# Newiz430/CellSegmentation

Measured on AMD Instinct MI355X. Metric: tiles/sec fwd+bwd (ResNet-50 MIL, 299x299), higher is better.
Workload: dtype bf16; 1 GPU; ResNet-50 tile classifier (train_tile.py --scratch semantics: fwd + CE + full bwd + Adam), bag=64 tiles of 299x299x3 per GPU, freeze_bn=True; tiles_per_gpu=64, parallelism=dp1

## Files before the change

### cellsegmentation_amd/_lib.py

```python
import ctypes
import os
from ctypes import POINTER, Structure, c_char_p, c_double, c_float, c_int, c_int32, c_int64, c_longlong, c_size_t, c_void_p

_HERE = os.path.dirname(os.path.abspath(__file__))
FLAVOUR = os.environ.get("CELLSEG_LIB_FLAVOUR", "")
if FLAVOUR not in ("", "ab"):
    raise RuntimeError(f"CELLSEG_LIB_FLAVOUR={FLAVOUR!r}: expected unset or 'ab'")
LIB_PATH = os.path.join(_HERE, f"libcellseg_hip_{FLAVOUR}.so" if FLAVOUR else "libcellseg_hip.so")

CS_F32, CS_BF16 = 0, 1
CS_ACT_NONE, CS_ACT_RELU, CS_ACT_SILU, CS_ACT_SIGMOID = 0, 1, 2, 3
CS_BN_BWD_OWN_RELU, CS_BN_BWD_FROZEN = 0x100, 0x200


class CsConvGeom(Structure):
    _fields_ = [(n, c_int32) for n in ("N", "H", "W", "C", "K", "R", "S", "stride", "pad", "P", "Q", "groups")]


class CsStageDesc(Structure):
    _fields_ = ([(n, c_void_p) for n in ("w", "gamma", "beta", "mean", "var", "conv_bias", "w_khwc", "w_chwk", "scale", "shift", "rstd")]
                + [("eps", c_float)] + [(n, c_int32) for n in ("K", "Cin", "R", "S", "Cp", "Kp", "block0", "fwd_packed", "bwd_packed")])


class CellsegLibraryMissing(RuntimeError):
# ... 15 lines not shown
    "cs_stage_conv_bn_multi": (c_int, [_P, c_int, c_int, c_int, _P]),
    "cs_stage_conv_bn_one": (c_int, [POINTER(CsStageDesc), c_int, _P]),
    "cs_weight_prep": (c_int, [_P, _P, c_int, c_int, c_int, c_int, c_int, c_int, c_int, _P, _P, _P]),
    "cs_conv2d_fwd": (c_int, [POINTER(CsConvGeom), c_int, _P, _P, _P, _P, _P, c_int, _P, _P, _P, _P]),
    "cs_conv2d_stats_workspace": (c_size_t, [c_longlong, c_int]),
    "cs_igemm_tile": (c_int, [c_longlong, c_int]),
    "cs_conv2d_dgrad": (c_int, [POINTER(CsConvGeom), c_int, _P, _P, _P, _P, _P, _P, _P, _P]),
    "cs_conv2d_fwd_bits": (c_int, [POINTER(CsConvGeom), c_int, _P, _P, _P, _P, _P, c_int, _P, _P, _P]),
    "cs_conv2d_dgrad_bits": (c_int, [POINTER(CsConvGeom), c_int, _P, _P, _P, _P, _P, _P, _P, _P]),
    "cs_conv2d_packed_supported": (c_int, [POINTER(CsConvGeom), c_int]),
    "cs_conv2d_packed_weight_bytes": (c_size_t, [POINTER(CsConvGeom), c_int]),
    "cs_pack_conv_weights": (c_int, [POINTER(CsConvGeom), c_int, _P, _P, _P]),
    "cs_conv2d_packed_partial_rows": (c_int, [POINTER(CsConvGeom), c_int]),
    "cs_conv2d_fwd_packed": (c_int, [POINTER(CsConvGeom), _P, _P, _P, _P, c_int, _P, _P, _P]),
    "cs_conv2d_dgrad_packed": (c_int, [POINTER(CsConvGeom), _P, _P, _P, c_int, _P, _P, _P, _P]),
    "cs_conv2d_wgrad": (c_int, [POINTER(CsConvGeom), c_int, _P, _P, _P, c_int, _P]),
    "cs_wgrad_finalize": (c_int, [_P, c_int, c_int, _P, _P, _P, _P, _P, c_int, c_int, c_int, c_int, c_int, _P, _P, _P, _P, _P, c_int, _P]),
    "cs_conv2d_wgrad_splits": (c_int, [POINTER(CsConvGeom), c_int]),
    "cs_weight_prep_grouped": (c_int, [_P, _P, c_int, c_int, c_int, c_int, c_int, _P, _P, _P]),
    "cs_conv2d_wgrad_batched_splits": (c_int, [POINTER(CsConvGeom), c_int, c_int]),
    "cs_conv2d_wgrad2_supported": (c_int, [POINTER(CsConvGeom), c_int]),
    "cs_conv2d_wgrad_batched": (c_int, [POINTER(CsConvGeom), c_int, _P, _P, _P, c_int, c_int, _P]),
    "cs_wgrad_finalize_batched": (c_int, [_P, _P, c_int, c_int, c_int, c_int, c_int, c_int, c_int, c_int, c_int, c_int, _P]),
    "cs_conv2d_dgrad_partial_rows": (c_int, [POINTER(CsConvGeom)]),
    "cs_fold_partial_rows": (c_int, [_P, c_int, c_int, _P, _P]),
    "cs_wgrad_finalize_grouped": (c_int, [_P, c_int, _P, _P, _P, _P, _P, c_int, c_int, c_int, c_int, _P, _P, _P, _P, _P]),
    "cs_colsum": (c_int, [_P, c_int, c_longlong, c_int, _P, _P]),
    "cs_colsum_partial_rows": (c_int, [c_longlong]),
    "cs_colsum_partial": (c_int, [_P, c_int, c_longlong, c_int, _P, _P]),
    "cs_positive_bits": (c_int, [_P, c_int, c_longlong, c_int, _P, _P]),
# ... 183 lines not shown
```

### cellsegmentation_amd/csrc/conv_v2.hip

```cpp
#include "cs_common.h"
#include <stdio.h>
#include <stdlib.h>
#include <utility>

namespace {

typedef int i32x4 __attribute__((ext_vector_type(4)));
typedef unsigned u32x4 __attribute__((ext_vector_type(4)));
constexpr unsigned OOB = 0x80000000u;

struct C2Params {
    const void* src;
    const void* wpk;
    void* dst;
    const float* shift;
    const void* residual;
    unsigned char* bits_out;
    const unsigned char* bits_in;
    float* slab;
    int act;
    int SH, SW, SC, NS;
    int DH, DW, NOUT;
    int Wp, Hp, PW, PH;
    int LW;
    int TH, TWl, tiles_x, tiles_y;
    unsigned n_tiles;
    int stride;
    int gather, GH, GWp;
    unsigned tap_sh[9];
    int lin;
    unsigned chunk_bytes;
    int add_stride, AH, AW;
    unsigned mg_dw, sh_dw, mg_dh, sh_dh, mg_wp, sh_wp, mg_hp, sh_hp;
    int NCC;
    int n_ntiles;
    unsigned M;
    unsigned src_bytes;
    unsigned pix_bytes;
    unsigned wpk_bytes;
};

__device__ __forceinline__ unsigned udivm(unsigned n, unsigned mg, unsigned sh) { return __umulhi(n, mg) >> sh; }

__device__ __forceinline__ i32x4 make_rsrc(const void* base, unsigned bytes) {
    const unsigned long long a = (unsigned long long)base;
    i32x4 r;
    r.x = (int)(unsigned)a;
    r.y = (int)((unsigned)(a >> 32) & 0xffffu);
    r.z = (int)bytes;
    r.w = 0x00020000;
    return r;
}
__device__ __forceinline__ unsigned lds_off(const void* p) { return (unsigned)(size_t)(__attribute__((address_space(3))) const unsigned char*)p; }

// ... 765 lines not shown
        wait_vm<0>();
        raw_barrier();
        epi.scr = smem_base + (unsigned)wave * EPI_WAVE;
    }
    asm volatile("s_nop 15\n\ts_nop 15\n\ts_nop 7");
    for_n<TM>([&]<int i>() {
        const f32x16 d = acc_read_w<i>();
        epi.template operator()<i>(d);
    });
    epi.finish();
    wait_vm<0>();
}

constexpr int R_MB = 96;

template <int TM, bool DG> struct RingEpilogue {
    static constexpr int E_OPS = 5 * TM + (DG ? 2 : 0);
    const C2Params& p;
    unsigned m0w = 0, m0w_next = 0xffffffffu, slab_row = 0;
    int n_w;
    bool alive;
    unsigned region;
    float sh[16];
    float s1[8];
    i32x4 q_res, q_bin;
    __amdgpu_buffer_rsrc_t r_dst, r_bout, r_slab;

    __device__ __forceinline__ RingEpilogue(const C2Params& p_, int n_w_, bool alive_, unsigned region_) : p(p_), n_w(n_w_), alive(alive_), region(region_) {}

    __device__ __forceinline__ unsigned piece() const {
        const unsigned lane = threadIdx.x & 63;
        return (lane & 3u) ^ ((lane >> 4) & 3u);
    }
    TileOffs cur, nxt;
    __device__ __forceinline__ void set_tile(unsigned base, unsigned base_next) {
        m0w = base; m0w_next = base_next;
        cur.set(base, alive, (unsigned)p.NOUT, (unsigned)n_w, piece(), p.M);
        nxt.set(base_next, alive, (unsigned)p.NOUT, (unsigned)n_w, piece(), p.M);
// ... 29 lines not shown

    __device__ __forceinline__ void prefetch(unsigned first_base) {
        const unsigned out_bytes = p.M * (unsigned)p.NOUT * 2u;
        r_dst = __builtin_amdgcn_make_buffer_rsrc(p.dst, 0, out_bytes, 0x00020000);
        r_bout = __builtin_amdgcn_make_buffer_rsrc(p.bits_out, 0, p.bits_out ? out_bytes >> 4 : 0u, 0x00020000);
        r_slab = __builtin_amdgcn_make_buffer_rsrc(p.slab, 0, p.slab ? 0x7ffffff0u : 0u, 0x00020000);
        q_res = make_rsrc(p.residual, !p.residual ? 0u : p.add_stride == 1 ? out_bytes : (unsigned)(p.NS * p.AH * p.AW * p.NOUT) * 2u);
        q_bin = make_rsrc(p.bits_in, p.bits_in ? out_bytes >> 4 : 0u);
        const int hh = (threadIdx.x & 63) >> 5;
#pragma unroll
        for (int g = 0; g < 4; ++g) {
            float4 s = make_float4(0.f, 0.f, 0.f, 0.f);
            if (!DG && p.shift && alive) s = *reinterpret_cast<const float4*>(p.shift + n_w + 8 * g + 4 * hh);
            sh[4 * g] = s.x; sh[4 * g + 1] = s.y; sh[4 * g + 2] = s.z; sh[4 * g + 3] = s.w;
        }
#pragma unroll
        for (int r = 0; r < 16; ++r) asm volatile("" : "+v"(sh[r]));
        TileOffs first;
        first.set(first_base, alive, (unsigned)p.NOUT, (unsigned)n_w, piece(), p.M);
        arm_all(first, std::make_integer_sequence<int, TM>{});
    }

    template <int I> __device__ __forceinline__ void operator()(const f32x16& acc) {
        const int lane = threadIdx.x & 63;
        const unsigned pc = piece();
        float v[16];
#pragma unroll
        for (int r = 0; r < 16; ++r) v[r] = DG ? acc[r] : acc[r] + sh[r];
        if (p.residual) {
            const uint4 xa = lds_get(acc_lds(I, 0)), xb = lds_get(acc_lds(I, 1));
            __builtin_amdgcn_wave_barrier();
            add_residual(v, xa, xb);
        }
        unsigned pk[8];
        pack_tile(v, !DG && p.act == CS_ACT_RELU, pk);
        lds_put(acc_lds(I, 0), make_uint4(pk[0], pk[1], pk[2], pk[3]));
        lds_put(acc_lds(I, 1), make_uint4(pk[4], pk[5], pk[6], pk[7]));
        __builtin_amdgcn_wave_barrier();
        uint4 o0 = lds_get(row_lds(I, 0)), o1 = lds_get(row_lds(I, 1));
        __builtin_amdgcn_wave_barrier();
        asm volatile("" : "+v"(o0.x), "+v"(o1.w));
        if constexpr (DG) {
            if (p.bits_in) {
                unsigned mbw;
// ... 24 lines not shown
                float a = s1[k];
                a += __shfl_xor(a, 4, 64);
                a += __shfl_xor(a, 8, 64);
                float t = a;
#pragma unroll
                for (int g = 1; g < 4; ++g) t += __shfl(a, ((lane & 3) ^ g) | (g << 4), 64);
                s1[k] = t;
            }
            const unsigned off = (lane < 4 && alive && p.slab) ? ((slab_row * 2u * (unsigned)p.NOUT + (unsigned)n_w + 8u * (unsigned)lane) * 4u) : OOB;
            __builtin_amdgcn_raw_buffer_store_b128(__builtin_bit_cast(u32x4, make_float4(s1[0], s1[1], s1[2], s1[3])), r_slab, off, 0, 0);
            __builtin_amdgcn_raw_buffer_store_b128(__builtin_bit_cast(u32x4, make_float4(s1[4], s1[5], s1[6], s1[7])), r_slab, off, 16, 0);
        }
    }
};

template <int TM, int WM, int WN, bool DG, bool GA = false>
__global__ __launch_bounds__(256, 2) __attribute__((amdgpu_num_vgpr(48))) void conv2_ring_kernel(C2Params p, int n_groups) {
    static_assert(WM * WN == 4 && WM * TM <= 4 && TM >= 2, "a ring slot holds up to 128 pixel rows");
    constexpr int BM = WM * TM * 32, BN = WN * 32;
    constexpr unsigned SLOT = 16384u, NSLOT = 3u, SLOT_ROWS = 128u;
    using Epi = RingEpilogue<TM, DG>;
    constexpr int E = Epi::E_OPS;
    static_assert(12 + 2 * E <= 63, "vmcnt field");
    extern __shared__ __attribute__((aligned(16))) unsigned char smem[];

    const int tid = threadIdx.x, lane = tid & 63;
    const int wave = __builtin_amdgcn_readfirstlane(tid >> 6);
    const int wm = wave / WN, wn = wave % WN;
    const int l31 = lane & 31, hh = lane >> 5;
    const WgTile wg(p);
    const unsigned group = wg.mtile;
    const int n_w = wg.n_w(p, BN, wn);
    const bool alive = n_w < p.NOUT;
    if (group * BM >= p.M) return;
    const int NCC = p.NCC;

    unsigned qb[4];
#pragma unroll
    for (int i = 0; i < 4; ++i) qb[i] = (unsigned)((wm * TM + (i < TM ? i : 0)) * 32 + l31);
    const i32x4 rsrc_a = make_rsrc(p.src, p.src_bytes);
    const i32x4 rsrc_b = make_rsrc(p.wpk, p.wpk_bytes);
    const unsigned smem_base = lds_off(smem);
    const unsigned hhb = (unsigned)hh * 256u;
    const unsigned cf0 = 0xf0u;
    const unsigned w_base = (unsigned)(n_w >> 5) * (unsigned)NCC * 4096u;

    int f_gy[2] = {0, 0}, f_gx[2] = {0, 0};
    auto tile_voff = [&](unsigned mt, unsigned (&vo)[2]) {
#pragma unroll
        for (int j = 0; j < 2; ++j) {
            const unsigned m = mt * BM + 16u * (unsigned)(wave + 4 * j) + (unsigned)(lane & 15);
            if (BM < 128 && 16 * (wave + 4 * j) >= BM) { vo[j] = OOB; continue; }
            if constexpr (GA) {
                const unsigned yall = udivm(m, p.mg_dw, p.sh_dw);
                const unsigned x = m - yall * (unsigned)p.DW;
                const unsigned n = udivm(yall, p.mg_dh, p.sh_dh);
                const unsigned y = yall - n * (unsigned)p.DH;
                vo[j] = (m < p.M && mt != 0xffffffffu) ? n * (unsigned)(p.GH * p.GWp) * 16u : 0xffffffffu;
                f_gy[j] = 2 * (int)y - 3;
                f_gx[j] = (int)x - 2;
                continue;
            }
            unsigned pix = m;
            if (p.stride > 1) {
                const unsigned yall = udivm(m, p.mg_dw, p.sh_dw);
                const unsigned x = m - yall * (unsigned)p.DW;
                const unsigned n = udivm(yall, p.mg_dh, p.sh_dh);
                const unsigned y = yall - n * (unsigned)p.DH;
                pix = (n * (unsigned)p.SH + y * (unsigned)p.stride) * (unsigned)p.SW + x * (unsigned)p.stride;
            }
            vo[j] = (m < p.M && mt != 0xffffffffu) ? pix * p.pix_bytes + (unsigned)(lane >> 4) * 16u : OOB;
        }
    };

    Epi epi(p, n_w, alive, smem_base + NSLOT * SLOT + (unsigned)wave * (unsigned)(TM * 2048));
    unsigned mt = group;
    epi.prefetch(mt * BM + (unsigned)(wm * TM * 32));
    asm volatile("; v[96:255] are owned by the main loop" ::: "v96", "v255");
    vzero_seq(std::make_integer_sequence<int, 16 * TM>{});

    unsigned f_mt = mt, f_slot = 0;
    int f_c = 0;
    unsigned f_vo[2];
    tile_voff(f_mt, f_vo);
    auto advance_fetch = [&]() {
        f_slot = f_slot == NSLOT - 1 ? 0u : f_slot + 1u;
        if (++f_c == NCC) {
            f_c = 0;
            if (f_mt != 0xffffffffu) {
                f_mt += (unsigned)n_groups;
                if (f_mt * BM >= p.M) f_mt = 0xffffffffu;
            }
            tile_voff(f_mt, f_vo);
        }
    };
    auto issue_b = [&]<int J>() {
        const unsigned bv = (alive && f_mt != 0xffffffffu) ? (unsigned)lane * 16u : OOB;
        bload4<J>(rsrc_b, bv, w_base + (unsigned)f_c * 4096u);
    };
    auto issue_a = [&]() {
        const unsigned dst = smem_base + f_slot * SLOT;
        if constexpr (GA) {
#pragma unroll
            for (int j = 0; j < 2; ++j) {
                auto slot_off = [&](int sl) -> unsigned {
                    const int kh = sl >> 2, pw = sl & 3;
                    const int iy = f_gy[j] + kh, px = f_gx[j] + pw;
                    const bool ok = f_vo[j] != 0xffffffffu && sl < 28 && (unsigned)iy < (unsigned)p.GH && (unsigned)px < (unsigned)p.GWp;
                    return ok ? f_vo[j] + (unsigned)(iy * p.GWp + px) * 16u : OOB;
                };
                const int s0 = f_c * 8 + (lane >> 4);
                dma_block2(rsrc_a, dst + (unsigned)(wave + 4 * j) * 2048u, slot_off(s0), slot_off(s0 + 4));
            }
            return;
        }
        dma_block(rsrc_a, dst + (unsigned)wave * 2048u, f_vo[0], (unsigned)f_c * 128u);
        dma_block(rsrc_a, dst + (unsigned)(wave + 4) * 2048u, f_vo[1], (unsigned)f_c * 128u);
    };
    issue_b.template operator()<0>(); issue_a(); advance_fetch();
    issue_b.template operator()<1>(); issue_a(); advance_fetch();
    int c = 0;
    unsigned slot = 0;
    bool fin1 = false, fin2 = false;
    auto step = [&]<int CUR>() -> bool {
        issue_b.template operator()<(CUR + 2) % 3>();
        const int nfin = (int)fin1 + (int)fin2;
        if (nfin == 0) wait_vm<12>();
        else if (nfin == 1) wait_vm<12 + E>();
        else wait_vm<12 + 2 * E>();
        raw_barrier();
        issue_a();
        advance_fetch();
        const unsigned sh_cur = slot * SLOT_ROWS;
        const bool fin = c == NCC - 1;
        bool more = true;
        if (!fin) {
            tap_mfma<TM, CUR, 0, 0u, 0u, true, false, true, false>(qb[0], qb[1], qb[2], qb[3], sh_cur, 0u, hhb, cf0);
            ++c;
        } else {
            const unsigned mt_next = mt + (unsigned)n_groups;
            const bool has_next = mt_next * BM < p.M;
            epi.set_tile(mt * BM + (unsigned)(wm * TM * 32), has_next ? mt_next * BM + (unsigned)(wm * TM * 32) : 0xffffffffu);
            epi.slab_row = mt * WM + wm;
            auto on_tile = [&]<int i>(const f32x16& d) {
                if (NCC == 1) wait_vm_mem<(E - 5 + 8 < 63 ? E - 5 + 8 : 63)>();
                else if (NCC == 2) wait_vm_mem<(E - 5 + 16 < 63 ? E - 5 + 16 : 63)>();
                epi.template operator()<i>(d);
            };
            tap_mfma<TM, CUR, 0, 0u, 0u, true, false, true, true>(qb[0], qb[1], qb[2], qb[3], sh_cur, 0u, hhb, cf0, on_tile);
            epi.finish();
            vzero_seq(std::make_integer_sequence<int, 16 * TM>{});
// ... 213 lines not shown
    static const int ring_tm = cs_env_int_("CELLSEG_RING_TM", 0);
    pl.tm = pl.kind == C2Kind::Ring22 ? 2 : (ring_tm >= 2 && ring_tm <= 4) ? ring_tm : pick_tm(p.M, p.n_ntiles);
    pl.nbw = 0;
    if (pl.kind == C2Kind::Ring14 && p.stride == 1 && !compact && p.NCC % 4 == 0) {
        const int wtm = pick_wide1_tm(p.M, p.n_ntiles, p.NCC);
        if (wtm) {
            pl.kind = C2Kind::Wide1x1; pl.tm = wtm; pl.nbw = wtm;
            p.lin = 1; p.chunk_bytes = 256u;
            p.tap_sh[0] = 0u; p.tap_sh[1] = 32u * (unsigned)wtm;
        }
    }
    pl.rows = partial_rows(pl);
    return true;
}

template <typename F, typename... Args>
int launch_kernel(F fn, const char* name, unsigned grid, size_t lds, hipStream_t st, const Args&... args) {
    if (!cs_allow_dynamic_lds_(reinterpret_cast<const void*>(fn), lds, lds > 81920 ? 163840 : 81920)) return CS_ERR_LAUNCH;
    cs_set_variant_(name);
    hipLaunchKernelGGL(fn, dim3(grid), dim3(256), lds, st, args...);
    CS_LAUNCH_CHECK();
    return CS_OK;
}
const char* tf(bool b) { return b ? "true" : "false"; }
unsigned xcd_grid(unsigned n_mt, int n_ntiles) { return ((n_mt + 7) / 8) * 8 * (unsigned)n_ntiles; }

template <int TM, int WM, int WN, bool DG>
int launch_ring_t(const C2Params& p, hipStream_t st) {
    const unsigned n_mt = (unsigned)cs_ceil_div(p.M, 32 * TM * WM);
    const unsigned best = ring_groups(n_mt, (unsigned)p.n_ntiles, nullptr);
    const size_t lds = 3 * 16384 + 4 * (size_t)TM * 2048;
    char name[64];
    snprintf(name, sizeof(name), "conv2_ring_kernel<%d,%d,%d,%s,%s>", TM, WM, WN, tf(DG), tf(p.gather));
    if constexpr (TM == 2 && !DG) {
        if (p.gather) return launch_kernel(conv2_ring_kernel<TM, WM, WN, DG, true>, name, best * (unsigned)p.n_ntiles, lds, st, p, (int)best);
    }
    if (p.gather) {
        cs_set_error_("conv2: gathered operand rows are served for 64 output channels only");
        return CS_ERR_UNSUPPORTED;
    }
    return launch_kernel(conv2_ring_kernel<TM, WM, WN, DG>, name, best * (unsigned)p.n_ntiles, lds, st, p, (int)best);
}

template <int TM, int WM, int WN, int NBW, bool DG, bool T2D = false>
int launch_halo_t(const C2Params& p, hipStream_t st) {
    const unsigned n_mt = T2D ? p.n_tiles : (unsigned)cs_ceil_div(p.M, 32 * TM * WM);
    const size_t lds = NBW != 8 && p.NCC > 1 ? (size_t)NBW * 8192 * 2 : (size_t)NBW * 8192 + EPI_LDS;
    char name[64];
    snprintf(name, sizeof(name), "conv2_halo_kernel<9,3,%d,%d,%d,%d,%s,%s>", TM, WM, WN, NBW, tf(DG), tf(T2D));
    return launch_kernel(conv2_halo_kernel<9, 3, TM, WM, WN, NBW, DG, T2D>, name, xcd_grid(n_mt, p.n_ntiles), lds, st, p);
}

template <int TM, int NBW, bool DG, int NTAP>
int launch_wide_t(const C2Params& p, hipStream_t st) {
    const unsigned n_mt = (unsigned)cs_ceil_div(p.M, 32 * TM);
    const size_t lds = (size_t)NBW * 8192 * (NTAP == 9 ? 2 : 3);
// ... 74 lines not shown
extern "C" int cs_conv2d_fwd_packed(const CsConvGeom* g, const void* x, const void* w_packed, const float* shift, const void* residual, int act,
                                    void* y, uint8_t* positive_bits, void* stream) {
    CS_CHECK_ARG(g && x && w_packed && y, "conv2d_fwd_packed: NULL tensor");
    CS_CHECK_ARG(act == CS_ACT_NONE || act == CS_ACT_RELU, "conv2d_fwd_packed: activation must be none or ReLU");
    C2Plan pl;
    if (!plan_any(g, 0, pl)) {
        cs_set_error_("conv2d_fwd_packed: geometry not served by the packed-operand kernel (ask cs_conv2d_packed_supported first)");
        return CS_ERR_UNSUPPORTED;
    }
    pl.p.src = x; pl.p.wpk = w_packed; pl.p.dst = y;
    pl.p.shift = shift; pl.p.residual = residual; pl.p.act = act;
    pl.p.bits_out = positive_bits;
    return launch_plan(pl, reinterpret_cast<hipStream_t>(stream), false);
}

extern "C" int cs_conv2d_dgrad_packed(const CsConvGeom* g, const void* dy, const void* w_packed, const void* add, int add_stride,
                                      const uint8_t* mask_bits, void* dx, float* partial_rows, void* stream) {
    CS_CHECK_ARG(g && dy && w_packed && dx, "conv2d_dgrad_packed: NULL tensor");
    CS_CHECK_ARG(add_stride == 1 || (add_stride == 2 && add), "conv2d_dgrad_packed: add_stride is 1, or 2 with a compact add operand");
    C2Plan pl;
    if (!plan_any(g, 1, pl)) {
        cs_set_error_("conv2d_dgrad_packed: geometry not served by the packed-operand kernel (ask cs_conv2d_packed_supported first)");
        return CS_ERR_UNSUPPORTED;
    }
    if (g->stride != 1)
        CS_CHECK_ARG(!add && !mask_bits && !partial_rows,
                     "conv2d_dgrad_packed: a strided 1x1 data gradient is written in compact [N][P][Q][C] form, without add / mask / column sums");
    if (add_stride == 2) {
        CS_CHECK_ARG(is_1x1(pl.kind) && pl.p.DH >= 2 && pl.p.DW >= 2, "conv2d_dgrad_packed: a strided add operand is served by the 1x1 kernels only");
        pl.p.add_stride = 2;
// ... 27 lines not shown
```

### cellsegmentation_amd/engine.py

```python
from collections import namedtuple
from types import SimpleNamespace

import torch

from . import _capture
from . import kernels as K

ACT_NONE, ACT_RELU, ACT_SILU = K.CS_ACT_NONE, K.CS_ACT_RELU, K.CS_ACT_SILU

PACKED = True
PACKED_TRAIN_BN = True
FUSE_STEM_POOL = True


class ConvUnit:
    kind = "conv"

    def __init__(self, name, conv, bn, act, src, dst, res=None):
        self.name, self.conv, self.bn, self.act = name, conv, bn, act
        self.src, self.dst, self.res = src, dst, res
        self.grouped = conv.groups != 1
        if self.grouped:
            cg = conv.in_channels // conv.groups
            if conv.in_channels != conv.out_channels or conv.in_channels % 64 != 0 or 64 % cg != 0 or conv.bias is not None:
                raise NotImplementedError(f"{name}: grouped convolution needs C == K, C % 64 == 0, (C/groups) | 64, no bias "
                                          "(the ResNeXt 32x4d / 32x8d 3x3 layers)")
        self._cache = None
# ... 4 lines not shown
            out.append(("bias", self.conv.bias))
        if self.bn is not None:
            out += [("gamma", self.bn.weight), ("beta", self.bn.bias)]
        return out

    def inputs(self):
        return [self.src] + ([self.res] if self.res is not None else [])

    def fwd(self, f, ui):
        x = f.t[self.src]
        N, H, W, Cp = x.shape
        conv = self.conv
        Kp = K.pad_channels(conv.out_channels)
        R, S = conv.kernel_size
        geom = K.make_geom(N, H, W, Cp, Kp, R, S, conv.stride[0], conv.padding[0])
        res = f.t[self.res] if self.res is not None else None
        batch_stats = _bn_uses_batch_stats(self.bn, f.bn_train)
        st = f.staged(ui, self, geom, batch_stats)
        stem = _is_paired_stem(self) and K.is_stem_geom(geom)
        xp = wp = None
        if ui == 0 and f.nchw_for_stem is not None:
            if not stem:
                raise RuntimeError("engine: the stem was expected to take the NCHW image (placeholder input would be read)")
            xp = K.stem_pair_from_nchw(f.nchw_for_stem, f.dtype)
        elif stem:
            xp = K.stem_pair_input(x)
        if stem:
            wp = K.stem_pair_weights(st.w_khwc)
        if batch_stats:
            stats = f.take_stats(Kp)
            if stem:
                z = K.stem_fwd(geom, xp, wp, None, st.shift, ACT_NONE, stats=stats)
            elif st.fwd_packed:
                z = K.conv_fwd_packed(geom, x, st.w_khwc, st.shift, None, ACT_NONE)
                K.bn_stats(z, stats)
            else:
                z = K.conv_fwd(geom, x, st.w_khwc, None, st.shift, None, ACT_NONE, stats=stats, grouped=self.grouped)
            y, mean, rstd = f.bn_train_fwd(self.bn, z, stats, res, self.act)
            f.aux[ui] = SimpleNamespace(geom=geom, st=st, train=True, z=z if f.save else None, mean=mean, rstd=rstd, xp=xp)
        else:
            want_bits = f.save and self.act == ACT_RELU
            pool_ui = None
            if stem and PACKED and FUSE_STEM_POOL and self.act == ACT_RELU and K.stem_pool_fwd_supported(geom, f.dtype):
                pool_ui = _sole_pool_consumer(f.plan, self)
            if pool_ui is not None:
                f.t[f.plan.units[pool_ui].dst], am = K.stem_pool_fwd(geom, xp, wp, st.shift, want_argmax=f.save)
                f.aux[pool_ui] = SimpleNamespace(argmax=am, in_hw=(geom.P, geom.Q))
                f.aux[ui] = SimpleNamespace(geom=geom, st=st, train=False, xp=xp)
                return
            if stem and PACKED and K.stem_fwd_packed_supported(geom, f.dtype):
                y = K.stem_fwd_packed(geom, xp, K.stem_pack_weights(wp), st.shift, self.act)
            elif stem:
                y = K.stem_fwd(geom, xp, wp, None, st.shift, self.act)
            elif st.fwd_packed and want_bits:
                y, f.bits[self.dst] = K.conv_fwd_packed(geom, x, st.w_khwc, st.shift, res, self.act, want_bits=True)
            elif st.fwd_packed:
# ... 248 lines not shown
def _is_paired_stem(u):
    if u.kind != "conv":
        return False
    c = u.conv
    return (not u.grouped and u.res is None and c.in_channels <= 3 and c.kernel_size == (7, 7)
            and c.stride == (2, 2) and c.padding == (3, 3))


def _sole_pool_consumer(plan, u):
    if plan.consumers.get(u.dst, 0) != 1 or u.dst in plan.outputs:
        return None
    for vi, v in enumerate(plan.units):
        if u.dst in v.inputs():
            return vi if v.kind == "pool" else None
    return None


def _stem_takes_nchw(plan, dtype):
    if not (dtype == torch.bfloat16 and len(plan.inputs) == 1 and plan.units):
        return False
    u = plan.units[0]
    return (_is_paired_stem(u) and u.conv.in_channels == 3 and u.src == plan.inputs[0]
            and plan.consumers.get(u.src, 0) == 1)


def _packed_flags(plan, u, geom, dtype, need_bwd, batch_stats, bits, bn_train=False):
    if not PACKED or u.grouped or u.act not in (ACT_NONE, ACT_RELU):
        return False, False
    if batch_stats:
        if not (PACKED_TRAIN_BN and geom.R == 3 and geom.S == 3 and geom.stride == 1 and min(geom.C, geom.K) >= 128):
# ... 113 lines not shown
            if pack is not None and pack.valid():
                pack.launch()
                self.prestaged = pack.by_unit
                if self.capturing:
                    _capture.keep(pack)
            else:
                self.packs.pop(self.pack_key, None)
                while len(self.packs) >= 4:
                    self.packs.pop(next(iter(self.packs)))
                self.record = []

        self.bumped = []
        if bn_train and save:
            K.begin_pass(dev)
        self.bits = {}
        n_stats = sum(K.accum_words(K.pad_channels(u.conv.out_channels)) for u in plan.units
                      if u.kind == "conv" and _bn_uses_batch_stats(u.bn, bn_train)) if bn_train else 0
        self.stats = _Arena(n_stats, torch.float64, dev, 1)
        self.dw_hwc = self._stage_depthwise()

    def _stage_depthwise(self):
        plan = self.plan
        units = [ui for ui, u in enumerate(plan.units) if u.kind == "dw"]
        if not units:
            return {}
        ws = [plan.units[ui].conv.weight.detach() for ui in units]
        if not all(w.is_contiguous() and w.dtype == torch.float32 and w.dim() == 4 and w.shape[1] == 1 for w in ws):
            return {}
        dpack = plan.__dict__.get("_dw_stage_pack")
        if dpack is None or dpack.key != tuple(w.data_ptr() for w in ws):
# ... 324 lines not shown
```

### cellsegmentation_amd/kernels.py

```python
import ctypes

import torch

from . import _lib
from ._lib import (CS_ACT_NONE, CS_ACT_RELU, CS_ACT_SIGMOID, CS_ACT_SILU, CS_BF16, CS_BN_BWD_FROZEN, CS_BN_BWD_OWN_RELU, CS_F32,
                   CsConvGeom)


def _code(dtype):
    if dtype == torch.float32:
        return CS_F32
    if dtype == torch.bfloat16:
        return CS_BF16
    raise TypeError(f"unsupported activation dtype {dtype}; use torch.float32 or torch.bfloat16")


def _f32(*tensors):
    for t in tensors:
        if t.dtype != torch.float32:
            raise TypeError(f"this kernel reads torch.float32 only, got {t.dtype}; cast on the way in (functional.py does)")


def chunk(dtype):
    return 4 if dtype == torch.float32 else 8
# ... 232 lines not shown
    lib = _lib.load()
    n = lib.cs_conv2d_packed_weight_bytes(ctypes.byref(geom), 1 if dgrad else 0) // 2
    if out is None:
        out = torch.empty((n,), dtype=torch.bfloat16, device=w_staged.device)
    _lib.check(lib.cs_pack_conv_weights(ctypes.byref(geom), 1 if dgrad else 0, _p(w_staged), _p(out), _stream()), "pack_conv_weights")
    return out


def conv_fwd_packed(geom, x, w_packed, shift=None, residual=None, act=CS_ACT_NONE, want_bits=False, out=None):
    y = out if out is not None else torch.empty((geom.N, geom.P, geom.Q, geom.K), dtype=x.dtype, device=x.device)
    bits = torch.empty((geom.N, geom.P, geom.Q, geom.K // 8), dtype=torch.uint8, device=x.device) if want_bits else None
    lib = _lib.load()
    _lib.check(_timed("fwd", geom, x.dtype, lambda: lib.cs_conv2d_fwd_packed(
        ctypes.byref(geom), _p(x), _p(w_packed), _p(shift), _p(residual), act, _p(y), _p(bits), _stream()),
        extra_tensors=int(residual is not None) + (1.0 / 16 if want_bits else 0.0)), "conv2d_fwd_packed")
    return (y, bits) if want_bits else y


class CompactGrad:

    def __init__(self, t, stride):
        self.t, self.stride = t, stride


def conv_dgrad_packed(geom, dy, w_packed, add=None, mask_bits=None, want_colsum=False):
    lib = _lib.load()
    if geom.stride != 1:
        if add is not None or mask_bits is not None or want_colsum:
            raise ValueError("conv_dgrad_packed: a strided 1x1 data gradient is compact -- no add, mask or column sums")
        dxc = torch.empty((geom.N, geom.P, geom.Q, geom.C), dtype=dy.dtype, device=dy.device)
# ... 1744 lines not shown
```

### include/cellseg_hip.h

```cpp
#ifndef CELLSEG_HIP_H_
#define CELLSEG_HIP_H_

#include <stdint.h>
#include <stddef.h>

#ifdef __cplusplus
extern "C" {
#endif

enum { CS_F32 = 0, CS_BF16 = 1 };
enum { CS_OK = 0, CS_ERR_INVALID_ARG = -1, CS_ERR_LAUNCH = -2, CS_ERR_UNSUPPORTED = -3 };
enum { CS_ACT_NONE = 0, CS_ACT_RELU = 1, CS_ACT_SILU = 2, CS_ACT_SIGMOID = 3 };

int cs_abi_version(void);
const char* cs_last_error(void);
const char* cs_last_conv_variant(void);

typedef struct CsConvGeom {
    int32_t N, H, W, C;
    int32_t K;
    int32_t R, S;
    int32_t stride, pad;
    int32_t P, Q;
    int32_t groups;
// ... 158 lines not shown
                           void* stream);

size_t cs_segmented_topk_workspace(long long T);
int cs_segmented_topk(const float* probs, const int32_t* groups, const int32_t* k_per_tile,
                      const int64_t* seg_offsets, int n_groups, int max_run, long long T, int64_t* out_idx,
                      int64_t* out_count, void* workspace, size_t workspace_bytes, void* stream);

int cs_conv2d_packed_supported(const CsConvGeom* g, int dgrad);
size_t cs_conv2d_packed_weight_bytes(const CsConvGeom* g, int dgrad);
int cs_pack_conv_weights(const CsConvGeom* g, int dgrad, const void* w_staged, void* w_packed, void* stream);
int cs_conv2d_packed_partial_rows(const CsConvGeom* g, int dgrad);
int cs_conv2d_fwd_packed(const CsConvGeom* g, const void* x, const void* w_packed, const float* shift, const void* residual, int act,
                         void* y, uint8_t* positive_bits, void* stream);
int cs_conv2d_dgrad_packed(const CsConvGeom* g, const void* dy, const void* w_packed, const void* add, int add_stride,
                           const uint8_t* mask_bits, void* dx, float* partial_rows, void* stream);

int cs_stem_pair_input(const void* x_nhwc8, int dtype, int N, int H, int W, void* x_pair, void* stream);
int cs_stem_pair_from_nchw(const float* x_nchw, int dtype, int N, int H, int W, void* x_pair, void* stream);
int cs_stem_pair_weights(const void* w_khwc, int dtype, int K, void* w_pair, void* stream);
int cs_stem_fwd(int N, int H, int W, int K, int dtype, const void* x_pair, const void* w_pair, const float* scale, const float* shift,
                int act, void* y, double* stats, void* workspace, void* stream);
int cs_stem_fwd_packed(int N, int H, int W, int K, const void* x_pair, const void* w_packed, const float* shift, int act, void* y,
                       uint8_t* positive_bits, void* stream);
int cs_stem_pool_fwd_supported(int N, int H, int W, int K);
int cs_stem_pool_fwd(int N, int H, int W, int K, const void* x_pair, const void* w_pair, const float* shift, void* y_pool,
                     uint8_t* argmax, void* stream);
int cs_stem_wgrad_splits(int N, int H, int W, int K);
int cs_stem_wgrad(int N, int H, int W, int K, int dtype, const void* x_pair, const void* dy, float* dw_pair_slabs, int use_tr_read,
                  void* stream);
int cs_stem_unpair_slabs(const float* dw_pair_slabs, int nsplit, int K, float* dw_khwc, void* stream);
// ... 190 lines not shown
```

Measured before the change: 9543 tiles/s.

## Fuse ResNet downsample shortcut 1x1 conv into the block's final 1x1 conv

Adds a two-source ring conv kernel that first accumulates the shortcut 1x1 (optionally strided) conv, stashes its biased result in LDS, then runs the main 1x1 conv and adds the stash as the residual in the epilogue. The engine detects eligible shortcut/main pairs under frozen BN and routes the shortcut through the fused launch instead of materialising its output. This removes one kernel launch and a write plus read of the shortcut activation per bottleneck-with-downsample block. The cost is extra kernel complexity and register/LDS pressure, and the fusion applies only to the four downsample blocks in the forward pass.

```diff
diff --git a/cellsegmentation_amd/_lib.py b/cellsegmentation_amd/_lib.py
--- a/cellsegmentation_amd/_lib.py
+++ b/cellsegmentation_amd/_lib.py
@@ -53,6 +53,8 @@
     "cs_conv2d_packed_partial_rows": (c_int, [POINTER(CsConvGeom), c_int]),
     "cs_conv2d_fwd_packed": (c_int, [POINTER(CsConvGeom), _P, _P, _P, _P, c_int, _P, _P, _P]),
     "cs_conv2d_dgrad_packed": (c_int, [POINTER(CsConvGeom), _P, _P, _P, c_int, _P, _P, _P, _P]),
+    "cs_conv2d_fwd_shortcut_supported": (c_int, [POINTER(CsConvGeom), POINTER(CsConvGeom)]),
+    "cs_conv2d_fwd_shortcut_packed": (c_int, [POINTER(CsConvGeom), _P, _P, _P, POINTER(CsConvGeom), _P, _P, _P, c_int, _P, _P, _P]),
     "cs_conv2d_wgrad": (c_int, [POINTER(CsConvGeom), c_int, _P, _P, _P, c_int, _P]),
     "cs_wgrad_finalize": (c_int, [_P, c_int, c_int, _P, _P, _P, _P, _P, c_int, c_int, c_int, c_int, c_int, _P, _P, _P, _P, _P, c_int, _P]),
     "cs_conv2d_wgrad_splits": (c_int, [POINTER(CsConvGeom), c_int]),
diff --git a/cellsegmentation_amd/csrc/conv_v2.hip b/cellsegmentation_amd/csrc/conv_v2.hip
--- a/cellsegmentation_amd/csrc/conv_v2.hip
+++ b/cellsegmentation_amd/csrc/conv_v2.hip
@@ -38,6 +38,11 @@
     unsigned src_bytes;
     unsigned pix_bytes;
     unsigned wpk_bytes;
+    int NCC_a;
+    unsigned src2_bytes, pix2_bytes, wpk2_bytes;
+    const void* src2;
+    const void* wpk2;
+    const float* shift2;
 };
 
 __device__ __forceinline__ unsigned udivm(unsigned n, unsigned mg, unsigned sh) { return __umulhi(n, mg) >> sh; }
@@ -833,7 +838,9 @@
 
 constexpr int R_MB = 96;
 
-template <int TM, bool DG> struct RingEpilogue {
+struct NoShift2 {};
+struct Shift2 { float v[16]; };
+template <int TM, bool DG, bool S2 = false> struct RingEpilogue {
     static constexpr int E_OPS = 5 * TM + (DG ? 2 : 0);
     const C2Params& p;
     unsigned m0w = 0, m0w_next = 0xffffffffu, slab_row = 0;
@@ -841,6 +848,7 @@
     bool alive;
     unsigned region;
     float sh[16];
+    [[no_unique_address]] std::conditional_t<S2, Shift2, NoShift2> sh2;
     float s1[8];
     i32x4 q_res, q_bin;
     __amdgpu_buffer_rsrc_t r_dst, r_bout, r_slab;
@@ -900,6 +908,16 @@
             if (!DG && p.shift && alive) s = *reinterpret_cast<const float4*>(p.shift + n_w + 8 * g + 4 * hh);
             sh[4 * g] = s.x; sh[4 * g + 1] = s.y; sh[4 * g + 2] = s.z; sh[4 * g + 3] = s.w;
         }
+        if constexpr (S2) {
+#pragma unroll
+            for (int g = 0; g < 4; ++g) {
+                float4 s = make_float4(0.f, 0.f, 0.f, 0.f);
+                if (p.shift2 && alive) s = *reinterpret_cast<const float4*>(p.shift2 + n_w + 8 * g + 4 * hh);
+                sh2.v[4 * g] = s.x; sh2.v[4 * g + 1] = s.y; sh2.v[4 * g + 2] = s.z; sh2.v[4 * g + 3] = s.w;
+            }
+#pragma unroll
+            for (int r = 0; r < 16; ++r) asm volatile("" : "+v"(sh2.v[r]));
+        }
 #pragma unroll
         for (int r = 0; r < 16; ++r) asm volatile("" : "+v"(sh[r]));
         TileOffs first;
@@ -907,13 +925,24 @@
         arm_all(first, std::make_integer_sequence<int, TM>{});
     }
 
+    template <int I> __device__ __forceinline__ void stash(const f32x16& acc) {
+        float v[16];
+#pragma unroll
+        for (int r = 0; r < 16; ++r) v[r] = acc[r] + sh2.v[r];
+        unsigned pk[8];
+        pack_tile(v, false, pk);
+        lds_put(acc_lds(I, 0), make_uint4(pk[0], pk[1], pk[2], pk[3]));
+        lds_put(acc_lds(I, 1), make_uint4(pk[4], pk[5], pk[6], pk[7]));
+        __builtin_amdgcn_wave_barrier();
+    }
+
     template <int I> __device__ __forceinline__ void operator()(const f32x16& acc) {
         const int lane = threadIdx.x & 63;
         const unsigned pc = piece();
         float v[16];
 #pragma unroll
         for (int r = 0; r < 16; ++r) v[r] = DG ? acc[r] : acc[r] + sh[r];
-        if (p.residual) {
+        if (S2 || p.residual) {
             const uint4 xa = lds_get(acc_lds(I, 0)), xb = lds_get(acc_lds(I, 1));
             __builtin_amdgcn_wave_barrier();
             add_residual(v, xa, xb);
@@ -968,12 +997,13 @@
     }
 };
 
-template <int TM, int WM, int WN, bool DG, bool GA = false>
+template <int TM, int WM, int WN, bool DG, bool GA = false, bool S2 = false>
 __global__ __launch_bounds__(256, 2) __attribute__((amdgpu_num_vgpr(48))) void conv2_ring_kernel(C2Params p, int n_groups) {
     static_assert(WM * WN == 4 && WM * TM <= 4 && TM >= 2, "a ring slot holds up to 128 pixel rows");
+    static_assert(!S2 || (!DG && !GA && WM == 1), "two sources: forward, 1 x 4 waves, plain operand rows");
     constexpr int BM = WM * TM * 32, BN = WN * 32;
     constexpr unsigned SLOT = 16384u, NSLOT = 3u, SLOT_ROWS = 128u;
-    using Epi = RingEpilogue<TM, DG>;
+    using Epi = RingEpilogue<TM, DG, S2>;
     constexpr int E = Epi::E_OPS;
     static_assert(12 + 2 * E <= 63, "vmcnt field");
     extern __shared__ __attribute__((aligned(16))) unsigned char smem[];
@@ -997,10 +1027,14 @@
     const unsigned smem_base = lds_off(smem);
     const unsigned hhb = (unsigned)hh * 256u;
     const unsigned cf0 = 0xf0u;
-    const unsigned w_base = (unsigned)(n_w >> 5) * (unsigned)NCC * 4096u;
+    const int NCC_a = S2 ? p.NCC_a : NCC;
+    const unsigned w_base = (unsigned)(n_w >> 5) * (unsigned)NCC_a * 4096u;
+    const i32x4 rsrc_a2 = S2 ? make_rsrc(p.src2, p.src2_bytes) : rsrc_a;
+    const i32x4 rsrc_b2 = S2 ? make_rsrc(p.wpk2, p.wpk2_bytes) : rsrc_b;
+    const unsigned w_base2 = S2 ? (unsigned)(n_w >> 5) * (unsigned)(NCC - NCC_a) * 4096u : 0u;
 
     int f_gy[2] = {0, 0}, f_gx[2] = {0, 0};
-    auto tile_voff = [&](unsigned mt, unsigned (&vo)[2]) {
+    auto tile_voff = [&](unsigned mt, unsigned (&vo)[2], bool src_b = false) {
 #pragma unroll
         for (int j = 0; j < 2; ++j) {
             const unsigned m = mt * BM + 16u * (unsigned)(wave + 4 * j) + (unsigned)(lane & 15);
@@ -1016,6 +1050,12 @@
                 continue;
             }
             unsigned pix = m;
+            if constexpr (S2) {
+                if (src_b) {
+                    vo[j] = (m < p.M && mt != 0xffffffffu) ? m * p.pix2_bytes + (unsigned)(lane >> 4) * 16u : OOB;
+                    continue;
+                }
+            }
             if (p.stride > 1) {
                 const unsigned yall = udivm(m, p.mg_dw, p.sh_dw);
                 const unsigned x = m - yall * (unsigned)p.DW;
@@ -1039,6 +1079,13 @@
     tile_voff(f_mt, f_vo);
     auto advance_fetch = [&]() {
         f_slot = f_slot == NSLOT - 1 ? 0u : f_slot + 1u;
+        if constexpr (S2) {
+            if (f_c + 1 == NCC_a) {
+                ++f_c;
+                tile_voff(f_mt, f_vo, true);
+                return;
+            }
+        }
         if (++f_c == NCC) {
             f_c = 0;
             if (f_mt != 0xffffffffu) {
@@ -1050,6 +1097,12 @@
     };
     auto issue_b = [&]<int J>() {
         const unsigned bv = (alive && f_mt != 0xffffffffu) ? (unsigned)lane * 16u : OOB;
+        if constexpr (S2) {
+            if (f_c >= NCC_a) {
+                bload4<J>(rsrc_b2, bv, w_base2 + (unsigned)(f_c - NCC_a) * 4096u);
+                return;
+            }
+        }
         bload4<J>(rsrc_b, bv, w_base + (unsigned)f_c * 4096u);
     };
     auto issue_a = [&]() {
@@ -1067,6 +1120,13 @@
                 dma_block2(rsrc_a, dst + (unsigned)(wave + 4 * j) * 2048u, slot_off(s0), slot_off(s0 + 4));
             }
             return;
+        }
+        if constexpr (S2) {
+            if (f_c >= NCC_a) {
+                dma_block(rsrc_a2, dst + (unsigned)wave * 2048u, f_vo[0], (unsigned)(f_c - NCC_a) * 128u);
+                dma_block(rsrc_a2, dst + (unsigned)(wave + 4) * 2048u, f_vo[1], (unsigned)(f_c - NCC_a) * 128u);
+                return;
+            }
         }
         dma_block(rsrc_a, dst + (unsigned)wave * 2048u, f_vo[0], (unsigned)f_c * 128u);
         dma_block(rsrc_a, dst + (unsigned)(wave + 4) * 2048u, f_vo[1], (unsigned)f_c * 128u);
@@ -1088,7 +1148,18 @@
         const unsigned sh_cur = slot * SLOT_ROWS;
         const bool fin = c == NCC - 1;
         bool more = true;
-        if (!fin) {
+        if (S2 && c == NCC_a - 1) {
+            if constexpr (S2) {
+                auto on_stash = [&]<int i>(const f32x16& d) {
+                    if (NCC_a == 1) wait_vm_mem<8 + 5 * (TM - 1 - i)>();
+                    else if (NCC_a == 2) wait_vm_mem<16 + 5 * (TM - 1 - i)>();
+                    epi.template stash<i>(d);
+                };
+                tap_mfma<TM, CUR, 0, 0u, 0u, true, false, true, true>(qb[0], qb[1], qb[2], qb[3], sh_cur, 0u, hhb, cf0, on_stash);
+                vzero_seq(std::make_integer_sequence<int, 16 * TM>{});
+                ++c;
+            }
+        } else if (!fin) {
             tap_mfma<TM, CUR, 0, 0u, 0u, true, false, true, false>(qb[0], qb[1], qb[2], qb[3], sh_cur, 0u, hhb, cf0);
             ++c;
         } else {
@@ -1332,6 +1403,33 @@
     return true;
 }
 
+bool plan_shortcut(const CsConvGeom* a, const CsConvGeom* b, C2Plan& pl) {
+    for (const CsConvGeom* g : {a, b}) {
+        if (g->groups > 1 || g->R != 1 || g->S != 1 || g->pad != 0 || g->N < 1 || g->H < 1 || g->W < 1 || g->C < 64 || g->C % 64) return false;
+        if (g->stride < 1 || g->P != (g->H - 1) / g->stride + 1 || g->Q != (g->W - 1) / g->stride + 1) return false;
+    }
+    if (a->stride != 1 || (b->stride != 1 && b->stride != 2)) return false;
+    if (a->N != b->N || a->P != b->P || a->Q != b->Q || a->K != b->K) return false;
+    if (a->K < 128 || a->K % 128) return false;
+    if (b->stride > 1 && (a->P < 2 || a->Q < 2)) return false;
+    pl.kind = C2Kind::Ring14;
+    if (!fill_params(pl, b->N, b->H, b->W, b->C, (unsigned)b->C * 2u, b->P, b->Q, b->K, 1)) return false;
+    const unsigned long long src2_bytes = (unsigned long long)a->N * a->H * a->W * (unsigned long long)a->C * 2ull;
+    const unsigned long long wbytes2 = packed_weight_bytes(a->K, 1, a->C);
+    if (src2_bytes >= 0x80000000ull || wbytes2 >= 0x80000000ull) return false;
+    C2Params& p = pl.p;
+    p.stride = b->stride; p.add_stride = 1;
+    p.NCC_a = p.NCC;
+    p.NCC = p.NCC_a + a->C / 64;
+    p.src2_bytes = (unsigned)src2_bytes;
+    p.pix2_bytes = (unsigned)a->C * 2u;
+    p.wpk2_bytes = (unsigned)wbytes2;
+    pl.tm = pick_tm(p.M, p.n_ntiles);
+    pl.nbw = 0;
+    pl.rows = partial_rows(pl);
+    return true;
+}
+
 template <typename F, typename... Args>
 int launch_kernel(F fn, const char* name, unsigned grid, size_t lds, hipStream_t st, const Args&... args) {
     if (!cs_allow_dynamic_lds_(reinterpret_cast<const void*>(fn), lds, lds > 81920 ? 163840 : 81920)) return CS_ERR_LAUNCH;
@@ -1358,6 +1456,16 @@
         return CS_ERR_UNSUPPORTED;
     }
     return launch_kernel(conv2_ring_kernel<TM, WM, WN, DG>, name, best * (unsigned)p.n_ntiles, lds, st, p, (int)best);
+}
+
+template <int TM>
+int launch_ring2_t(const C2Params& p, hipStream_t st) {
+    const unsigned n_mt = (unsigned)cs_ceil_div(p.M, 32 * TM);
+    const unsigned best = ring_groups(n_mt, (unsigned)p.n_ntiles, nullptr);
+    const size_t lds = 3 * 16384 + 4 * (size_t)TM * 2048;
+    char name[64];
+    snprintf(name, sizeof(name), "conv2_ring_kernel<%d,1,4,false,false,true>", TM);
+    return launch_kernel(conv2_ring_kernel<TM, 1, 4, false, false, true>, name, best * (unsigned)p.n_ntiles, lds, st, p, (int)best);
 }
 
 template <int TM, int WM, int WN, int NBW, bool DG, bool T2D = false>
@@ -1462,6 +1570,32 @@
     return launch_plan(pl, reinterpret_cast<hipStream_t>(stream), false);
 }
 
+extern "C" int cs_conv2d_fwd_shortcut_supported(const CsConvGeom* main, const CsConvGeom* shortcut) {
+    if (!main || !shortcut) return 0;
+    C2Plan pl;
+    return plan_shortcut(main, shortcut, pl) ? 1 : 0;
+}
+
+extern "C" int cs_conv2d_fwd_shortcut_packed(const CsConvGeom* main, const void* x, const void* w_packed, const float* shift,
+                                             const CsConvGeom* shortcut, const void* x_in, const void* w_packed_sc, const float* shift_sc, int act,
+                                             void* y, uint8_t* positive_bits, void* stream) {
+    CS_CHECK_ARG(main && shortcut, "conv2d_fwd_shortcut_packed: NULL geometry");
+    CS_CHECK_ARG(x && w_packed && x_in && w_packed_sc && y, "conv2d_fwd_shortcut_packed: NULL tensor");
+    CS_CHECK_ARG(act == CS_ACT_NONE || act == CS_ACT_RELU, "conv2d_fwd_shortcut_packed: activation must be none or ReLU");
+    C2Plan pl;
+    if (!plan_shortcut(main, shortcut, pl)) {
+        cs_set_error_("conv2d_fwd_shortcut_packed: geometry pair not served (ask cs_conv2d_fwd_shortcut_supported first)");
+        return CS_ERR_UNSUPPORTED;
+    }
+    C2Params& p = pl.p;
+    p.src = x_in; p.wpk = w_packed_sc; p.shift2 = shift_sc;
+    p.src2 = x; p.wpk2 = w_packed; p.shift = shift;
+    p.dst = y; p.act = act; p.bits_out = positive_bits;
+    hipStream_t st = reinterpret_cast<hipStream_t>(stream);
+    if (pl.tm == 3) return launch_ring2_t<3>(p, st);
+    return launch_ring2_t<4>(p, st);
+}
+
 extern "C" int cs_conv2d_dgrad_packed(const CsConvGeom* g, const void* dy, const void* w_packed, const void* add, int add_stride,
                                       const uint8_t* mask_bits, void* dx, float* partial_rows, void* stream) {
     CS_CHECK_ARG(g && dy && w_packed && dx, "conv2d_dgrad_packed: NULL tensor");
diff --git a/cellsegmentation_amd/engine.py b/cellsegmentation_amd/engine.py
--- a/cellsegmentation_amd/engine.py
+++ b/cellsegmentation_amd/engine.py
@@ -11,6 +11,7 @@
 PACKED = True
 PACKED_TRAIN_BN = True
 FUSE_STEM_POOL = True
+FUSE_SHORTCUT = True
 
 
 class ConvUnit:
@@ -45,7 +46,8 @@
         Kp = K.pad_channels(conv.out_channels)
         R, S = conv.kernel_size
         geom = K.make_geom(N, H, W, Cp, Kp, R, S, conv.stride[0], conv.padding[0])
-        res = f.t[self.res] if self.res is not None else None
+        sc = f.fused_sc.pop(ui, None)
+        res = f.t[self.res] if (self.res is not None and sc is None) else None
         batch_stats = _bn_uses_batch_stats(self.bn, f.bn_train)
         st = f.staged(ui, self, geom, batch_stats)
         stem = _is_paired_stem(self) and K.is_stem_geom(geom)
@@ -71,6 +73,26 @@
             f.aux[ui] = SimpleNamespace(geom=geom, st=st, train=True, z=z if f.save else None, mean=mean, rstd=rstd, xp=xp)
         else:
             want_bits = f.save and self.act == ACT_RELU
+            main_ui = f.sc_pairs.get(ui)
+            if main_ui is not None and st.fwd_packed:
+                um = f.plan.units[main_ui]
+                zN, zH, zW, zC = f.t[um.src].shape
+                gm = K.make_geom(zN, zH, zW, zC, K.pad_channels(um.conv.out_channels), 1, 1, 1, 0)
+                main_packed = _packed_flags(f.plan, um, gm, f.dtype, False, False, f.bits, f.bn_train)[0]
+                if main_packed and K.conv_fwd_shortcut_supported(gm, geom, f.dtype):
+                    f.fused_sc[main_ui] = (geom, st, x)
+                    f.aux[ui] = SimpleNamespace(geom=geom, st=st, train=False, xp=None)
+                    return
+            if sc is not None:
+                if not st.fwd_packed:
+                    raise RuntimeError(f"{self.name}: a shortcut was left for this launch but its operand is not staged packed")
+                gv, stv, x_in = sc
+                y = K.conv_fwd_shortcut_packed(geom, x, st.w_khwc, st.shift, gv, x_in, stv.w_khwc, stv.shift, self.act, want_bits=want_bits)
+                if want_bits:
+                    y, f.bits[self.dst] = y
+                f.aux[ui] = SimpleNamespace(geom=geom, st=st, train=False, xp=None)
+                f.t[self.dst] = y
+                return
             pool_ui = None
             if stem and PACKED and FUSE_STEM_POOL and self.act == ACT_RELU and K.stem_pool_fwd_supported(geom, f.dtype):
                 pool_ui = _sole_pool_consumer(f.plan, self)
@@ -349,6 +371,43 @@
         if u.dst in v.inputs():
             return vi if v.kind == "pool" else None
     return None
+
+
+def shortcut_pairs(plan, bn_train):
+    if not (PACKED and FUSE_SHORTCUT):
+        return {}
+    key = (bool(bn_train), tuple(u.bn.training for u in plan.units if u.kind == "conv" and u.bn is not None))
+    cache = plan.__dict__.setdefault("_shortcut_pairs", {})
+    if key not in cache:
+        cache[key] = _find_shortcut_pairs(plan, bn_train)
+    return cache[key]
+
+
+def _find_shortcut_pairs(plan, bn_train):
+    producer = {v.dst: vi for vi, v in enumerate(plan.units) if v.kind == "conv"}
+    made_by = {w.dst: wi for wi, w in enumerate(plan.units)}
+    pairs = {}
+    for ui, u in enumerate(plan.units):
+        vi = producer.get(u.res) if u.kind == "conv" and u.res is not None else None
+        if vi is None or vi >= ui:
+            continue
+        v = plan.units[vi]
+
+        def one_by_one(w, strides):
+            c = w.conv
+            return not w.grouped and c.kernel_size == (1, 1) and c.padding == (0, 0) and c.stride in strides
+        if not (one_by_one(u, ((1, 1),)) and one_by_one(v, ((1, 1), (2, 2)))):
+            continue
+        if v.act != ACT_NONE or v.res is not None or u.act not in (ACT_NONE, ACT_RELU):
+            continue
+        if plan.consumers.get(v.dst, 0) != 1 or v.dst in plan.outputs:
+            continue
+        if u.src not in plan.inputs and made_by.get(u.src, len(plan.units)) >= vi:
+            continue
+        if _bn_uses_batch_stats(u.bn, bn_train) or _bn_uses_batch_stats(v.bn, bn_train):
+            continue
+        pairs[vi] = ui
+    return pairs
 
 
 def _stem_takes_nchw(plan, dtype):
@@ -492,6 +551,8 @@
         if bn_train and save:
             K.begin_pass(dev)
         self.bits = {}
+        self.sc_pairs = shortcut_pairs(plan, bn_train) if dtype == torch.bfloat16 else {}
+        self.fused_sc = {}
         n_stats = sum(K.accum_words(K.pad_channels(u.conv.out_channels)) for u in plan.units
                       if u.kind == "conv" and _bn_uses_batch_stats(u.bn, bn_train)) if bn_train else 0
         self.stats = _Arena(n_stats, torch.float64, dev, 1)
diff --git a/cellsegmentation_amd/kernels.py b/cellsegmentation_amd/kernels.py
--- a/cellsegmentation_amd/kernels.py
+++ b/cellsegmentation_amd/kernels.py
@@ -270,6 +270,20 @@
     _lib.check(_timed("fwd", geom, x.dtype, lambda: lib.cs_conv2d_fwd_packed(
         ctypes.byref(geom), _p(x), _p(w_packed), _p(shift), _p(residual), act, _p(y), _p(bits), _stream()),
         extra_tensors=int(residual is not None) + (1.0 / 16 if want_bits else 0.0)), "conv2d_fwd_packed")
+    return (y, bits) if want_bits else y
+
+
+def conv_fwd_shortcut_supported(geom, geom_sc, dtype):
+    return dtype == torch.bfloat16 and bool(_lib.load().cs_conv2d_fwd_shortcut_supported(ctypes.byref(geom), ctypes.byref(geom_sc)))
+
+
+def conv_fwd_shortcut_packed(geom, x, w_packed, shift, geom_sc, x_in, w_packed_sc, shift_sc, act=CS_ACT_NONE, want_bits=False, out=None):
+    y = out if out is not None else torch.empty((geom.N, geom.P, geom.Q, geom.K), dtype=x.dtype, device=x.device)
+    bits = torch.empty((geom.N, geom.P, geom.Q, geom.K // 8), dtype=torch.uint8, device=x.device) if want_bits else None
+    lib = _lib.load()
+    _lib.check(_timed("fwd", geom, x.dtype, lambda: lib.cs_conv2d_fwd_shortcut_packed(
+        ctypes.byref(geom), _p(x), _p(w_packed), _p(shift), ctypes.byref(geom_sc), _p(x_in), _p(w_packed_sc), _p(shift_sc), act, _p(y), _p(bits),
+        _stream()), extra_tensors=1.0 / 16 if want_bits else 0.0), "conv2d_fwd_shortcut_packed")
     return (y, bits) if want_bits else y
 
 
diff --git a/include/cellseg_hip.h b/include/cellseg_hip.h
--- a/include/cellseg_hip.h
+++ b/include/cellseg_hip.h
@@ -196,6 +196,10 @@
                          void* y, uint8_t* positive_bits, void* stream);
 int cs_conv2d_dgrad_packed(const CsConvGeom* g, const void* dy, const void* w_packed, const void* add, int add_stride,
                            const uint8_t* mask_bits, void* dx, float* partial_rows, void* stream);
+int cs_conv2d_fwd_shortcut_supported(const CsConvGeom* main, const CsConvGeom* shortcut);
+int cs_conv2d_fwd_shortcut_packed(const CsConvGeom* main, const void* x, const void* w_packed, const float* shift,
+                                  const CsConvGeom* shortcut, const void* x_in, const void* w_packed_sc, const float* shift_sc, int act,
+                                  void* y, uint8_t* positive_bits, void* stream);
 
 int cs_stem_pair_input(const void* x_nhwc8, int dtype, int N, int H, int W, void* x_pair, void* stream);
 int cs_stem_pair_from_nchw(const float* x_nchw, int dtype, int N, int H, int W, void* x_pair, void* stream);
```

Measured after the change: 9701 tiles/s, median of 6. 1.02x the previous value.
